# NilsJochem/audio-matcher

Measured on AMD Instinct MI355X. Metric: audio samples/s matched (whole node), 10 s needle vs 1 h haystack, 1/2/4/8 GPU, higher is better.
Workload: dtype f32

## Files before the change

### audio-matcher_amd/csrc/am_context.hip

```cpp
#include "am_internal.h"

namespace am {

thread_local std::string t_err;

int fail(int code, const std::string& msg) {
    t_err = msg;
    return code;
}
int hip_fail(hipError_t e, const char* what) {
    char buf[256];
    snprintf(buf, sizeof(buf), "%s: %s", what, hipGetErrorString(e));
    t_err = buf;
    return e == hipErrorOutOfMemory ? AM_ERR_OOM : AM_ERR_HIP;
}

static std::mutex g_hooks_mu;
static Hooks g_hooks;
Hooks snapshot_hooks() {
    std::lock_guard<std::mutex> lk(g_hooks_mu);
    return g_hooks;
}

using OptRule = const char* (*)(long long& v);
static const char* opt_any(long long&) { return nullptr; }
static const char* opt_bool(long long& v) { v = v ? 1 : 0; return nullptr; }
static const char* opt_log_n(long long& v) { return v != 0 && (v < kLogNMin || v > kLogNMax) ? "log_n out of range" : nullptr; }
static const char* opt_half(long long& v) { v = v <= 0 ? 0 : (v >= 2 ? 2 : 1); return nullptr; }
static const char* opt_every(long long& v) { v = v < 1 ? 1 : v; return nullptr; }
static const char* opt_arm_at(long long& v) { v = v < -1 ? -2 : v; return nullptr; }
static const char* opt_needle_group(long long& v) { return v < 1 || v > kMaxNeedleGroup ? "needle_group out of range" : nullptr; }
static const char* opt_pairs(long long& v) { return v < 1 || v > 64 ? "pairs_per_group out of range" : nullptr; }
static const char* opt_score_norm(long long& v) { return v < 0 || v > 1 ? "score_norm out of range (0 = off, 1 = NCC)" : nullptr; }
static const char* opt_floor_db(long long& v) { return v < 0 || v > 200 ? "score_norm_floor_db out of range (0..200)" : nullptr; }
static const char* opt_distance(long long& v) {
    return v < 0 || v > 3 ? "distance_rule out of range (bit 0: inclusive, bit 1: between plateau starts)" : nullptr;
}
struct Option {
    const char* name;
    std::atomic<long long> value;
    OptRule rule;
    long long Opts::*field;
};
static Option g_options[] = {
    {"log_n", {0}, opt_log_n, &Opts::log_n},
    {"pairs_per_group", {64}, opt_pairs, &Opts::pairs_per_group},
    {"profile_mask", {-1}, opt_any, &Opts::profile_mask},
    {"profile_every", {1}, opt_every, &Opts::profile_every},
    {"half_pipeline", {0}, opt_half, &Opts::half},
    {"batch_overlap", {1}, opt_bool, &Opts::batch_overlap},
    {"needle_group", {8}, opt_needle_group, &Opts::needle_group},
    {"pick_stream_priority", {0}, opt_bool, &Opts::pick_priority},
    {"pick_group", {1}, opt_bool, &Opts::pick_group},
    {"k3_group", {1}, opt_bool, &Opts::k3_group},
    {"host_pick_wait", {1}, opt_bool, &Opts::host_pick_wait},
    {"device_redo", {1}, opt_bool, &Opts::device_redo},
    {"tail_block", {1}, opt_bool, &Opts::tail_block},
    {"dense_scores", {0}, opt_bool, &Opts::dense},
    {"score_norm", {0}, opt_score_norm, &Opts::score_norm},
    {"score_norm_floor_db", {60}, opt_floor_db, &Opts::score_norm_floor_db},
    {"debug_no_realloc", {0}, opt_bool, &Opts::debug_no_realloc},
    {"debug_redo_arm_at", {-2}, opt_arm_at, &Opts::debug_redo_arm_at},
    {"peak_filter_order", {0}, opt_bool, &Opts::peak_filter_order},
    {"distance_rule", {0}, opt_distance, &Opts::distance_rule},
    {"tail_window", {0}, opt_bool, &Opts::tail_window},
    {"surrounding_from", {0}, opt_bool, &Opts::surrounding_from},
};
static Option* find_option(const char* key) {
    for (Option& r : g_options)
        if (!strcmp(key, r.name)) return &r;
    return nullptr;
}

thread_local const Opts* t_opts_pin = nullptr;
Opts snapshot_opts(const am_needle* h) {
    if (t_opts_pin) return *t_opts_pin;
    Opts o;
    for (const Option& r : g_options) o.*r.field = r.value.load(std::memory_order_relaxed);
    if (h && h->opt_log_n >= 0) o.log_n = h->opt_log_n;
    if (h && h->opt_half >= 0) o.half = h->opt_half;
    if (h && h->opt_score_norm >= 0) o.score_norm = h->opt_score_norm;
    return o;
}

thread_local int t_no_realloc = 0;
int realloc_refused(const char* what, size_t bytes, size_t cap) {
    char buf[160];
    snprintf(buf, sizeof(buf), "debug_no_realloc: %s buffer would grow from %zu to %zu bytes while a call is queueing", what, cap, bytes);
    return fail(AM_ERR_HIP, buf);
}

static const char* kKernelNames[] = {"k1_cols_fwd", "k2_rows", "k3_cols_inv", "tile_stats", "peaks", "other"};
static std::mutex g_ctx_mu;
static std::map<int, Ctx*> g_ctx;

int get_ctx(int device, Ctx** out) {
    std::lock_guard<std::mutex> lk(g_ctx_mu);
    int n = 0;
    hipError_t e = hipGetDeviceCount(&n);
    if (e != hipSuccess || n <= 0) return fail(AM_ERR_NO_DEVICE, "no HIP device available");
    if (device < 0 || device >= n) return fail(AM_ERR_NO_DEVICE, "device ordinal out of range");
    auto it = g_ctx.find(device);
    if (it != g_ctx.end()) { *out = it->second; AM_HIP(hipSetDevice(device)); return AM_OK; }
    AM_HIP(hipSetDevice(device));
    (void)hipSetDeviceFlags(hipDeviceScheduleSpin);
    (void)hipGetLastError();
    AM_HIP(fft_kernels_init());
    Ctx* c = new Ctx();
    c->device = device;
    c->hdr.flags = hipHostMallocMapped | hipHostMallocCoherent;
    c->failcnt.flags = hipHostMallocMapped | hipHostMallocCoherent;
    c->spill.flags = hipHostMallocMapped | hipHostMallocCoherent;
    hipError_t se = hipStreamCreateWithFlags(&c->stream, hipStreamNonBlocking);
    if (se != hipSuccess) { delete c; return hip_fail(se, "hipStreamCreate"); }
    {
        int least = 0, greatest = 0;
        if (snapshot_opts(nullptr).pick_priority && hipDeviceGetStreamPriorityRange(&least, &greatest) == hipSuccess && least != greatest)
            (void)hipStreamCreateWithPriority(&c->stream2, hipStreamNonBlocking, least);
        else
            (void)hipStreamCreateWithFlags(&c->stream2, hipStreamNonBlocking);
        (void)hipGetLastError();
    }
    (void)hipStreamCreateWithFlags(&c->stream_tail, hipStreamNonBlocking);
    (void)hipEventCreateWithFlags(&c->ev_fork, kSyncEvent);
    (void)hipEventCreateWithFlags(&c->ev_join, kSyncEvent);
    (void)hipGetLastError();
    for (int i = 0; i < 2; ++i) {
        (void)hipEventCreateWithFlags(&c->ev_k3[i], kSyncEvent);
        (void)hipEventCreateWithFlags(&c->ev_pick[i], kSyncEvent);
    }
    g_ctx[device] = c;
    *out = c;
    return AM_OK;
}

static hipEvent_t prof_event(Ctx* c) {
    if (!c->pool.empty()) { hipEvent_t e = c->pool.back(); c->pool.pop_back(); return e; }
    hipEvent_t e = nullptr;
// ... 445 lines not shown
```

### audio-matcher_amd/csrc/am_correlate.hip

```cpp
#include "am_internal.h"

namespace am {

static int pick_log_n(size_t s, long long out_count, const Opts& o, int* logN_out) {
    int min_log = kLogNMin;
    while (min_log <= kLogNMax && ((size_t)1 << min_log) < s + 1) ++min_log;
    if (min_log > kLogNMax) return fail(AM_ERR_INVALID_ARG, "needle too long for a forced transform size (2^23 at most; leave log_n at 0 for needle partitioning)");
    if (o.log_n > 0) {
        int l = (int)o.log_n;
        if (l < min_log) l = min_log;
        if (l > kLogNMax) l = kLogNMax;
        *logN_out = l;
        return AM_OK;
    }
    const long long span = out_count + (long long)s - 1;
    if (span > (1ll << 19)) {
        if ((long long)s <= kWideFromSamples) { *logN_out = 21; return AM_OK; }
        if ((long long)s <= kWidestFromSamples) {
            long long hop21 = (1ll << 21) - (long long)s + 1;
            if (hop21 >= 8 * kTile) hop21 = (hop21 / kTile) * kTile;
            *logN_out = (hop21 > 0 && out_count <= 2 * hop21) ? 21 : 22;
            return AM_OK;
        }
        if ((long long)s <= kSegmentFrom) {
// ... 154 lines not shown

int run_correlation(am_needle* h, const Opts& o, const void* d_src, long long src_len, long long lead,
                           float* d_dst, long long out_count, float factor,
                           const ScanRequest* scan_req, ScanResult* res, int src_kind, const PassPlan* plan) {
    int rc;
    PassPlan own;
    if (!plan) {
        if ((rc = pass_plan(h, o, out_count, scan_req && !scan_req->no_scan && lead == 0, &own))) return rc;
        plan = &own;
    }
    if (res) { res->fused = false; res->redo_ok = false; res->sparse = plain_scores(); }
    if (plan->kind != PassKind::Partitioned) return run_correlation_one(h, *plan, d_src, src_len, lead, d_dst, out_count, factor, scan_req, res, src_kind, false);
    if (scan_req && scan_req->skip_launch) return fail(AM_ERR_INVALID_ARG, "internal: streaming ingest does not run early pairs for partitioned needles");
    for (size_t i = 0; i < plan->parts.size(); ++i) {
        ScanRequest plain{};
        if (scan_req) {
            plain.margin = -1.0f; plain.range_a = scan_req->range_a; plain.range_b = scan_req->range_b;
            plain.before_k3 = i == 0 ? scan_req->before_k3 : nullptr;
            plain.no_scan = true;
        }
        if ((rc = run_correlation_one(h->segments[i], plan->parts[i], d_src, src_len, lead - h->seg_off[i], d_dst, out_count, factor,
                                      scan_req ? &plain : nullptr, nullptr, src_kind, i > 0)))
            return rc;
    }
    return AM_OK;
}

static int run_correlation_one(am_needle* h, const PassPlan& pp, const void* d_src, long long src_len, long long lead,
                               float* d_dst, long long out_count, float factor,
                               const ScanRequest* scan_req, ScanResult* res, int src_kind, bool accumulate) {
    Ctx* c = h->ctx;
    Job job{};
    job.src = d_src; job.src_len = src_len; job.lead = lead; job.src_kind = src_kind;
    job.dst = d_dst; job.out_count = out_count;
    if (pp.kind == PassKind::Direct) {
        ProfScope ps(c, KN_OTHER);
        AM_HIP(launch_direct(c->stream, job, h->d_needle, (int)h->n, factor));
        return AM_OK;
    }
    int rc;
    const PlanDev& pl = pp.pl->dev;
    const HalfScale& hs = pp.hs;
    const TailPlan& tail = pp.tail;
    const long long N = pp.g.N, hop = pp.g.hop, npairs = pp.npairs, ppg = pp.ppg;
    const ScanBuffers out = (scan_req && scan_req->out.work) ? scan_req->out : scan_buffers(c->side[0]);
    DevBuf& wk = *out.work;
    if ((rc = wk.ensure((size_t)ppg * (size_t)N * sizeof(float2)))) return rc;
    ScanCfg scan{};
    bool fused = false;
    if (scan_req && !scan_req->no_scan) {
        if (res) res->sparse = SparseScores{nullptr, nullptr, nullptr, (int)hop, pl.logN2, pl.logN1, 1.0 / (double)hop};
        if (pp.fused) {
            const long long side_blocks = std::max(pp.g.nblocks, scan_req->side_nblocks);
            if ((rc = out.stats32->ensure((size_t)((out_count + 31) / 32) * sizeof(float2)))) return rc;
            if ((rc = out.wflags->ensure(sparse_bytes(side_blocks, pl)))) return rc;
            fill_scan_cfg(&scan, out.stats32->p, out.wflags->p, side_blocks, pl, scan_req->margin, scan_req->hist_min, scan_req->seg_c, scan_req->seg_d);
            fused = true;
            if (res) { res->fused = true; res->sparse = sparse_view(scan, hop, pl); }
        }
    }
    const float k3scale = hs.k3(factor);
    job.out_count = pp.main_count; job.hop = (int)hop; job.nblocks = (int)pp.nblocks;
    if (scan_req && scan_req->skip_launch) return AM_OK;
    long long pair_lo = 0, pair_hi = npairs;
    bool with_tail = tail.on;
    if (scan_req && scan_req->range_b > scan_req->range_a) {
        pair_lo = (scan_req->range_a / hop) / 2;
        pair_hi = std::min(npairs, ((scan_req->range_b - 1) / hop) / 2 + 1);
        with_tail = tail.on && scan_req->range_b > tail.T;
    }
    if (scan_req && scan_req->tail_by_caller) with_tail = false;
    if (with_tail) {
        AM_HIP(hipEventRecord(c->ev_fork, c->stream));
        AM_HIP(hipStreamWaitEvent(c->stream_tail, c->ev_fork, 0));
        if ((rc = run_tail_block(c, pp, d_src, src_len, d_dst, out_count, factor, scan, src_kind))) return rc;
        AM_HIP(hipEventRecord(c->ev_join, c->stream_tail));
    }
    bool waited = false;
    for (long long first = pair_lo; first < pair_hi; first += ppg) {
        const int np = (int)std::min(ppg, pair_hi - first);
        job.first_pair = (int)first;
        { ProfScope ps(c, KN_K1); AM_HIP(launch_k1(c->stream, job, np, (float2*)wk.p, pl, hs.level)); }
        { ProfScope ps(c, KN_K2); AM_HIP(launch_k2(c->stream, np, (float2*)wk.p, pp.hc, pl, nullptr, hs.level, hs.hscale, hs.pre)); }
        if (!waited && scan_req && scan_req->before_k3) AM_HIP(hipStreamWaitEvent(c->stream, scan_req->before_k3, 0));
        waited = true;
        { ProfScope ps(c, KN_K3); AM_HIP(launch_k3(c->stream, job, np, (const float2*)wk.p, pl, k3scale, scan, hs.level, accumulate)); }
    }
    if (with_tail) AM_HIP(hipStreamWaitEvent(c->stream, c->ev_join, 0));
    if (res && fused && !accumulate && pair_lo == 0 && pair_hi == npairs && npairs <= ppg) {
        res->redo_ok = true;
        job.first_pair = 0;
        res->redo_job = job; res->redo_pl = pl; res->redo_scale = k3scale; res->redo_half = hs.level;
        res->redo_npairs = (int)npairs; res->redo_work = (const float2*)wk.p; res->redo_cfg = scan;
    }
    return AM_OK;
}

float scale_factor(const am_needle* h, int scale, size_t w) {
    if (scale == AM_SCALE_LIB) return h->inv_autocorr;
    if (scale == AM_SCALE_MY) return h->inv_autocorr / (float)w;
    return 1.0f;
}

static uint64_t start_nanos(uint64_t start, uint32_t sr) {
    const double t = (double)start / (double)sr;
    if (!(t > 0.0)) return 0;
    int e = 0;
    const double m = std::frexp(t, &e);
    const unsigned long long mant = (unsigned long long)std::ldexp(m, 53);
    const int sh = e - 53;
    unsigned __int128 v = (unsigned __int128)mant * 1000000000ull;
    if (sh >= 0) return (uint64_t)(v << sh);
    const int r = -sh;
    if (r >= 127) return 0;
    unsigned __int128 q = v >> r;
    const unsigned __int128 rem = v & (((unsigned __int128)1 << r) - 1);
    const unsigned __int128 half = (unsigned __int128)1 << (r - 1);
    if (rem > half || (rem == half && (q & 1))) ++q;
    return (uint64_t)q;
}

static bool is_overshadowed(const am_peak& element, const am_peak* other, uint32_t sr, double max_distance_s) {
    if (!other) return false;
    uint64_t e = start_nanos(element.start, sr), b = start_nanos(other->start, sr);
    if (e < b) std::swap(e, b);
    const uint64_t maxd = (uint64_t)std::llround(max_distance_s * 1e9);
    return (e - b) < maxd && other->prominence > element.prominence;
}

int upload_segments(Ctx* c, const std::vector<Segment>& segs) {
    const size_t bytes = sizeof(Segment) * segs.size();
    if (c->segs.p && segs.size() == c->segs_resident.size() &&
        memcmp(segs.data(), c->segs_resident.data(), bytes) == 0)
        return AM_OK;
    int rc;
    c->segs_resident.clear();
    if ((rc = c->segs.ensure(bytes))) return rc;
    if ((rc = c->pinned.ensure(bytes))) return rc;
    memcpy(c->pinned.p, segs.data(), bytes);
    AM_HIP(hipMemcpyAsync(c->segs.p, c->pinned.p, bytes, hipMemcpyHostToDevice, c->stream));
    AM_HIP(hipStreamSynchronize(c->stream));
    c->segs_resident = segs;
    return AM_OK;
}

int prepare_results(Ctx* c, size_t nhdr, size_t arena_entries, PeakArena* arena) {
    const size_t hdr_bytes = (sizeof(SegHeader) * nhdr + 63) / 64 * 64;
    int rc;
    if ((rc = c->hdr.ensure(hdr_bytes + sizeof(am_peak) * arena_entries))) return rc;
    if ((rc = c->arena_cur.ensure(sizeof(unsigned)))) return rc;
    AM_HIP(hipMemsetAsync(c->arena_cur.p, 0, sizeof(unsigned), c->stream));
    arena->base = reinterpret_cast<am_peak*>(static_cast<char*>(c->hdr.p) + hdr_bytes);
    arena->cursor = static_cast<unsigned*>(c->arena_cur.p);
    arena->cap = (unsigned)arena_entries;
    return AM_OK;
}

int wide_reserve(Ctx* c, size_t n) {
    int rc;
    if ((rc = c->wide_ctl.ensure(n * kWideCtlBytes))) return rc;
    if ((rc = c->wide_list.ensure(n * AM_MAX_PEAKS_PER_CHUNK * sizeof(am_peak)))) return rc;
    return c->wide_tiles.ensure(n * kWideTileList * sizeof(int));
}
WideState wide_carve(Ctx* c, size_t n) {
    WideState wide{};
    wide.best = static_cast<unsigned long long*>(c->wide_ctl.p);
    wide.state = reinterpret_cast<int*>(wide.best + n);
// ... 172 lines not shown
```

### audio-matcher_amd/csrc/am_engine.hip

```cpp
#include "am_internal.h"

namespace am {

static int launch_pick_group(Ctx* c, const K3Group& kg, long long n_scores, int seg_off, int nsegs, float min_prom, long long min_dist,
                             const SparseScores& sp_common, int* bad, const int* hdr_off, const PeakArena& arena, const PeakPolicy& pol,
                             hipStream_t st) {
    if (nsegs == 0 || n_scores <= 0 || kg.n <= 0) return AM_OK;
    int rc;
    const size_t nz = (size_t)kg.n, total = nz * (size_t)nsegs;
    const long long ntiles = (n_scores + kTile - 1) / kTile;
    PickGroup pg{};
    pg.n = kg.n;
    for (int z = 0; z < kg.n; ++z) {
        if ((rc = c->grp_stats[z].ensure((size_t)ntiles * sizeof(float2)))) return rc;
        pg.g[z] = kg.dst[z]; pg.stats[z] = static_cast<float2*>(c->grp_stats[z].p);
        pg.stats32[z] = kg.stats32[z]; pg.wbits[z] = kg.wbits[z]; pg.theta[z] = kg.tile_theta[z];
        pg.hdr_off[z] = hdr_off[z];
    }
    { ProfScope ps(c, KN_STATS, st);
      AM_HIP(launch_stats_reduce(st, pg.stats32[0], n_scores, pg.stats[0], bad, &pg)); }
    if ((rc = wide_reserve(c, total))) return rc;
    if ((rc = c->side[0].peaks.ensure(total * AM_MAX_PEAKS_PER_CHUNK * sizeof(am_peak)))) return rc;
    {
        ProfScope ps(c, KN_PEAKS, st);
        AM_HIP(launch_peaks(st, pg.g[0], n_scores, pg.stats[0], (const Segment*)c->segs.p + seg_off, nsegs, min_prom, min_dist,
                            (am_peak*)c->side[0].peaks.p, (SegHeader*)c->hdr.p, sp_common, arena, wide_carve(c, total), false, pol, &pg));
    }
    return AM_OK;
}


struct ChunkPlan {
    std::vector<Segment> segs, short_segs;
    std::vector<size_t> widths, short_w;
    std::vector<int> seg_off, short_off;
    std::vector<int> n_chunks;
    size_t max_scores = 0, max_segs = 1;
    int ns(size_t k) const { return seg_off[k + 1] - seg_off[k]; }
    bool too_many(size_t nn) const { return max_segs > (size_t)1 << 18 || segs.size() * nn > (size_t)1 << 24; }
};
static void plan_chunks(size_t s, const void* const* d_hays, const size_t* lens, size_t n_hay, const am_match_params* p, const Opts& o,
                        bool split_short, size_t max_windows, ChunkPlan* cp) {
    const size_t window = (size_t)(p->chunk + p->overlap);
    cp->seg_off.assign(n_hay + 1, 0);
    cp->short_off.assign(n_hay + 1, 0);
    cp->n_chunks.assign(n_hay, 0);
    for (size_t k = 0; k < n_hay; ++k) {
        cp->seg_off[k] = (int)cp->segs.size();
        cp->short_off[k] = (int)cp->short_segs.size();
        if (!d_hays[k] || lens[k] < s) continue;
        std::vector<Segment> one;
        std::vector<size_t> w1;
        make_segments(lens[k], s, p, o.tail_window != 0, one, &w1, max_windows);
        cp->n_chunks[k] = (int)one.size();
        for (size_t i = 0; i < one.size(); ++i) {
            const bool shorter = split_short && w1[i] != window;
            (shorter ? cp->short_segs : cp->segs).push_back(one[i]);
            (shorter ? cp->short_w : cp->widths).push_back(w1[i]);
        }
        if (!one.empty()) cp->max_scores = std::max(cp->max_scores, lens[k] - s + 1);
        cp->max_segs = std::max(cp->max_segs, cp->segs.size() - (size_t)cp->seg_off[k]);
    }
    cp->seg_off[n_hay] = (int)cp->segs.size();
    cp->short_off[n_hay] = (int)cp->short_segs.size();
}

struct ScoreSets {
    Ctx* c;
    bool overlap;
    size_t seq = 0;
    ScoreSets(Ctx* c_, const Opts& o, size_t n_items)
        : c(c_), overlap(o.batch_overlap && n_items > 1 && c_->stream2 && c_->ev_k3[0] && c_->ev_k3[1] && c_->ev_pick[0] && c_->ev_pick[1]) {}
    int count() const { return overlap ? 2 : 1; }
    int set() const { return overlap ? (int)(seq & 1) : 0; }
    ScoreSide& side() const { return c->side[set()]; }
    float* scores() const { return (float*)side().scores.p; }
    hipStream_t pick_stream() const { return overlap ? c->stream2 : c->stream; }
    int size(size_t max_scores, size_t max_segs) {
        int rc;
        for (int set = 0; set < count(); ++set) {
            ScoreSide& sd = c->side[set];
            if ((rc = sd.scores.ensure(max_scores * sizeof(float)))) return rc;
            if ((rc = sd.peaks.ensure(sizeof(am_peak) * max_segs * AM_MAX_PEAKS_PER_CHUNK))) return rc;
            if ((rc = sd.stats.ensure((max_scores + kTile - 1) / kTile * sizeof(float2)))) return rc;
        }
        return wide_reserve(c, max_segs);
    }
    int wait_pick(bool on_host) {
        if (!overlap || seq < 2) return AM_OK;
        if (on_host) AM_HIP(hipEventSynchronize(c->ev_pick[set()]));
        else AM_HIP(hipStreamWaitEvent(c->stream, c->ev_pick[set()], 0));
        return AM_OK;
    }
    int k3_done() {
        if (!overlap) return AM_OK;
        AM_HIP(hipEventRecord(c->ev_k3[set()], c->stream));
        AM_HIP(hipStreamWaitEvent(c->stream2, c->ev_k3[set()], 0));
        return AM_OK;
    }
    int pick_done() {
        if (overlap) AM_HIP(hipEventRecord(c->ev_pick[set()], c->stream2));
        ++seq;
        return AM_OK;
    }
    int drain() {
        AM_HIP(hipStreamSynchronize(c->stream));
        if (overlap) AM_HIP(hipStreamSynchronize(c->stream2));
        return AM_OK;
    }
};

static int match_alone(am_needle* h, const void* d_hay, size_t len, const am_match_params* p, am_peak* out, size_t cap, size_t slot,
                       size_t* n_out, int src_kind, const PartSpec* part, int* worst) {
    const int rc = match_many(h, &d_hay, &len, 1, p, out ? out + slot * cap : nullptr, cap, &n_out[slot], src_kind, 0, 1, false, nullptr, part);
    if (rc == AM_ERR_CAPACITY) *worst = rc;
    return rc == AM_ERR_CAPACITY ? AM_OK : rc;
}

static int pick_alone(am_needle* h, const Opts& o, const am_match_params* p, const void* src, long long src_len, float factor,
                      const ScanRequest& req, long long n_scores, int seg_idx, const Segment& sg, int spare_hdr, uint64_t shift, int src_kind,
                      const NormSpec& nrm, std::vector<am_peak>& all) {
    Ctx* c = h->ctx;
    const PeakPolicy pol = o.peak_policy();
    int rc;
    PeakArena own{};
    if ((rc = c->spill.ensure(sizeof(am_peak) * AM_MAX_PEAKS_PER_CHUNK))) return rc;
    AM_HIP(hipMemsetAsync(c->arena_cur.p, 0, sizeof(unsigned), c->stream));
    own.base = static_cast<am_peak*>(c->spill.p); own.cursor = static_cast<unsigned*>(c->arena_cur.p);
    own.cap = AM_MAX_PEAKS_PER_CHUNK;
    ScoreSide& side = c->side[0];
    if ((rc = side.scores.ensure((size_t)n_scores * sizeof(float)))) return rc;
    float* d_scores = (float*)side.scores.p;
    ScanResult res{};
    if ((rc = run_correlation(h, o, src, src_len, 0, d_scores, n_scores, factor, &req, &res, src_kind))) return rc;
    if (nrm.on) {
        if ((rc = normalise_scores(c, c->stream, nrm, src, src_len, src_kind, 0, (long long)h->n, d_scores, sg.a, std::min(sg.b, n_scores))))
            return rc;
        res.fused = false;
    }
    if ((rc = launch_pick(c, side, d_scores, n_scores, seg_idx, 1, p->min_prominence, (long long)p->min_distance, nullptr, &res, spare_hdr, own, pol))) return rc;
    AM_HIP(hipStreamSynchronize(c->stream));
    const SegHeader& hd = static_cast<const SegHeader*>(c->hdr.p)[spare_hdr];
    const size_t old = all.size();
    if (hd.overflow & 1) {
        if ((rc = pick_chunk_big(c, d_scores, n_scores, seg_idx, sg, p->min_prominence, (long long)p->min_distance, &res, hd.seg_min, all, pol)))
            return rc;
    } else append_header_peaks(hd, own, all);
    for (size_t j = old; j < all.size(); ++j) { all[j].start += shift; all[j].end += shift; }
    return AM_OK;
}

struct TailSlots { size_t scores, stats; };
static bool tail_batchable(const TailPlan& t) { return t.on && t.g.logN == 21; }
static int launch_tail_batch(am_needle* h, const std::vector<PassPlan>& plans, const std::vector<size_t>& members, int half_idx,
                             const TailSlots& sl, const void* const* d_hays, const size_t* lens, float factor, int src_kind) {
    Ctx* c = h->ctx;
    const PassPlan& lead = plans[members[0]];
    const TailPlan& first = lead.tail;
    const Plan* pl = lead.tail_pl;
    const float2* hc = lead.tail_hc;
    const HalfScale& hs = lead.tail_hs;
    TailBatch tb{};
    tb.n = (int)members.size();
    for (int j = 0; j < tb.n; ++j) {
        const size_t k = members[j];
        const size_t slot = (size_t)half_idx * kMaxTailBatch + (size_t)j;
        const Job job = tail_job(plans[k].tail, d_hays[k], (long long)lens[k], (long long)(lens[k] - h->n + 1), src_kind);
        tb.src[j] = job.src;
        tb.src_len[j] = job.src_len;
        tb.out_count[j] = job.out_count;
        tb.dst[j] = static_cast<float*>(c->tail_scores.p) + slot * sl.scores;
        tb.stats32[j] = static_cast<float2*>(c->tail_stats.p) + slot * sl.stats;
    }
    float2* work = static_cast<float2*>(c->work_tail.p);
    { ProfScope ps(c, KN_OTHER); AM_HIP(launch_tail_batch_k1(c->stream, tb, (int)first.g.hop, src_kind, work, pl->dev, hs.level)); }
    { ProfScope ps(c, KN_OTHER); AM_HIP(launch_k2(c->stream, tb.n, work, hc, pl->dev, nullptr, hs.level, hs.hscale, hs.pre, true)); }
    { ProfScope ps(c, KN_OTHER); AM_HIP(launch_tail_batch_k3(c->stream, tb, (int)first.g.hop, work, pl->dev, hs.k3(factor), hs.level)); }
    return AM_OK;
}

static int classify_nonfinite(am_needle* h, const PassPlan& pp, const float* d_hay, size_t len,
                              const std::vector<Segment>& segs, int s0, int s1,
                              std::vector<char>* drop, std::vector<char>* again) {
    Ctx* c = h->ctx;
    const long long s = (long long)h->n;
    const int nch = s1 - s0;
    drop->assign(nch, 0); again->assign(nch, 0);
    std::vector<Segment> ranges;
    for (int i = s0; i < s1; ++i)
        ranges.push_back(Segment{segs[i].a, std::min<long long>((long long)len, segs[i].b + s - 1)});
    const long long npairs = pp.kind == PassKind::Transform ? pp.npairs : 0;
    for (long long q = 0; q < npairs; ++q) ranges.push_back(pp.pair_reads(q, (long long)len));
    if (pp.tail.on) ranges.push_back(pp.tail_reads((long long)len));
    std::vector<int> flags(ranges.size(), 0);
    int rc = nonfinite_flags(c, d_hay, ranges.data(), (int)ranges.size(), flags.data());
    if (rc) return rc;
    for (int i = 0; i < nch; ++i) {
        if (flags[i]) { (*drop)[i] = 1; continue; }
        if (pp.kind == PassKind::Partitioned) { (*again)[i] = 1; continue; }
        const Segment sg = segs[s0 + i];
        for (long long q = 0; q < npairs && !(*again)[i]; ++q)
            if (flags[nch + q] && 2 * q * pp.g.hop < sg.b && (2 * q + 2) * pp.g.hop > sg.a) (*again)[i] = 1;
        if (pp.tail.on && flags[nch + npairs] && pp.tail.T < sg.b) (*again)[i] = 1;
    }
    return AM_OK;
}

int match_many(am_needle* h, const void* const* d_hays, const size_t* lens, size_t n_hay,
               const am_match_params* p, am_peak* out, size_t cap_per_hay, size_t* n_out, int src_kind,
               size_t index_base, size_t index_stride, bool fire_hooks, const StreamPre* pre, const PartSpec* part) {
    Ctx* c = h->ctx;
    const Opts o = snapshot_opts(h);
    const PeakPolicy pol = o.peak_policy();
    Hooks hooks = fire_hooks ? snapshot_hooks() : Hooks{};
    if (part) hooks.fn = nullptr;
    if (part && n_hay != 1) return fail(AM_ERR_INVALID_ARG, "internal: a part is one haystack");
    auto G = [&](size_t k) { return index_base + k * index_stride; };
    const size_t s = h->n;
    if (p->chunk == 0) return fail(AM_ERR_INVALID_ARG, "chunk must be > 0");
    if (p->scale < AM_SCALE_NONE || p->scale > AM_SCALE_MY) return fail(AM_ERR_INVALID_ARG, "bad scale");
    const NormSpec nrm = norm_spec(h, o);
    if (nrm.on && (pre || part)) return fail(AM_ERR_INVALID_ARG, AM_NORM_UNSUPPORTED);
    int rc = norm_check(nrm, p->scale);
    if (rc) return rc;
    const bool my = p->scale == AM_SCALE_MY;
    const float factor = nrm.on ? norm_factor(nrm) : scale_factor(h, p->scale, (size_t)(p->chunk + p->overlap));
    const int sm = p->scale == AM_SCALE_LIB ? 1 : 0;
    ScanRequest base{};
    base.margin = nrm.on ? -1.0f : write_margin(o, p);
    const bool sparse_ok = base.margin >= 0.0f;
    base.hist_min = nrm.on ? FLT_MAX : h->hist_min(sm);
    base.seg_c = (long long)p->chunk;
    base.seg_d = (long long)(p->chunk + p->overlap) - (long long)s;
    for (size_t k = 0; k < n_hay; ++k) n_out[G(k)] = 0;
    ChunkPlan cp;
    plan_chunks(s, d_hays, lens, n_hay, p, o, my, part ? part->max_windows : (size_t)-1, &cp);
    const std::vector<Segment>& segs = cp.segs;
    const std::vector<int>& seg_off = cp.seg_off;
    const size_t nsegs = segs.size();
    if (nsegs == 0 && cp.short_segs.empty()) return AM_OK;
    if (cp.too_many(1)) return fail(AM_ERR_INVALID_ARG, "chunk size too small for this haystack (more than 2^18 chunks)");
    size_t n_active = 0;
    for (size_t k = 0; k < n_hay; ++k) n_active += cp.ns(k) > 0;
    ScoreSets sets(c, o, n_active);
    if ((rc = sets.size(cp.max_scores, cp.max_segs))) return rc;
    std::vector<PassPlan> plans(n_hay);
    Footprint need;
    for (size_t k = 0; k < n_hay; ++k) {
        if (cp.n_chunks[k] == 0 || cp.ns(k) == 0) continue;
        if ((rc = pass_plan(h, o, (long long)(lens[k] - s + 1), pre == nullptr, &plans[k]))) return rc;
        need.take(plans[k].need);
    }
    std::vector<int> tail_slot(n_hay, -1);
    TailSlots tslots{0, 0};
    bool batch_tails = false;
    if (need.work_tail) {
        size_t n_tails = 0;
        for (size_t k = 0; k < n_hay; ++k)
            if (tail_batchable(plans[k].tail)) {
                ++n_tails;
                tslots.scores = std::max(tslots.scores, (size_t)(2 * plans[k].tail.g.hop));
            }
        tslots.stats = tslots.scores / 32;
        batch_tails = sets.overlap && n_tails > 1;
        const size_t nslot = batch_tails ? kMaxTailBatch : 1;
        if ((rc = c->work_tail.ensure(need.work_tail * nslot))) return rc;
        if (batch_tails) {
            if ((rc = c->tail_scores.ensure(2 * kMaxTailBatch * tslots.scores * sizeof(float)))) return rc;
            if ((rc = c->tail_stats.ensure(2 * kMaxTailBatch * tslots.stats * sizeof(float2)))) return rc;
        }
    }
    int tail_batches = 0;
    for (int set = 0; set < sets.count(); ++set) {
        if (need.work && (rc = c->side[set].work.ensure(need.work))) return rc;
        if (pre) continue;
        if (need.stats32 && (rc = c->side[set].stats32.ensure(need.stats32))) return rc;
        if (need.side && (rc = c->side[set].wflags.ensure(need.side))) return rc;
    }
    PeakArena arena{};
    if ((rc = prepare_results(c, nsegs + 1, std::min<size_t>(cp.max_segs * AM_MAX_PEAKS_PER_CHUNK, (size_t)1 << 20) + nsegs * 8, &arena))) return rc;
    std::vector<Segment> resident = segs;
    for (const Segment& sg : cp.short_segs) resident.push_back(Segment{0, sg.b - sg.a});
    const int local_seg = (int)resident.size();
    resident.push_back(Segment{0, std::max<long long>(base.seg_d + 1, 1)});
    if ((rc = upload_segments(c, resident))) return rc;
    if ((rc = c->badflag.ensure(sizeof(int) * n_hay))) return rc;
    int* h_bad = static_cast<int*>(c->badflag.p);
    memset(h_bad, 0, sizeof(int) * n_hay);
    if ((rc = c->failcnt.ensure(nsegs + 1))) return rc;
    if (nrm.on) {
        size_t max_len = 0;
        for (size_t k = 0; k < n_hay; ++k) if (cp.ns(k) > 0) max_len = std::max(max_len, lens[k]);
        if ((rc = norm_reserve(c, (long long)max_len))) return rc;
    }
    unsigned char* h_fail = static_cast<unsigned char*>(c->failcnt.p);
    memset(h_fail, 0, nsegs + 1);
    const bool device_redo = sets.overlap && sparse_ok && !needle_is_segmented(h, o) && o.device_redo != 0;
    if (device_redo) {
        for (int set = 0; set < 2; ++set)
            if ((rc = c->redo_pairs[set].ensure(sizeof(int) * (size_t)std::max<long long>(need.npairs, 1)))) return rc;
    }
    SegHeader* h_hdr = static_cast<SegHeader*>(c->hdr.p);
    auto chunk_events = [&](size_t k, int stage) {
        if (hooks.chunk_fn)
            for (int i = 0; i < cp.n_chunks[k]; ++i)
                hooks.chunk_fn(hooks.chunk_user, G(k), (part ? part->chunk_base : 0) + (size_t)i,
                               part ? part->chunk_total : (size_t)cp.n_chunks[k], stage);
    };
    const bool arm_forced = o.debug_redo_arm_at >= -1;
    bool redo_armed = device_redo && (arm_forced ? o.debug_redo_arm_at == 0 : h->redo_armed_left[sm] > 0);
    QueueingScope queueing(o.debug_no_realloc != 0);
    for (size_t k = 0; k < n_hay; ++k) {
        const int ns = cp.ns(k);
        if (cp.n_chunks[k] == 0) continue;
        if (device_redo && arm_forced) redo_armed = o.debug_redo_arm_at >= 0 && (long long)k >= o.debug_redo_arm_at;
        else if (device_redo && !redo_armed && (k & 3) == 0) {
            const volatile unsigned char* f = h_fail;
            for (int i = 0; i < seg_off[k] && !redo_armed; ++i) redo_armed = f[i] != 0;
        }
        if (hooks.fn) hooks.fn(hooks.user, G(k), 0, (size_t)cp.n_chunks[k]);
        chunk_events(k, 0);
        if (ns == 0) continue;
        const long long out_count = (long long)(lens[k] - s + 1);
        const int set = sets.set();
        const PassPlan& pp = plans[k];
        ScoreSide& side = sets.side();
        float* d_scores = sets.scores();
        ScanRequest req = base;
        req.out = scan_buffers(side);
        if ((rc = sets.wait_pick(o.host_pick_wait != 0))) return rc;
        int* d_redo = nullptr;
        if (redo_armed) {
            AM_HIP(hipMemsetAsync(c->redo_pairs[set].p, 0, sizeof(int) * (size_t)std::max<long long>(pp.g.npairs, 1), c->stream));
            d_redo = static_cast<int*>(c->redo_pairs[set].p);
        }
        int* bad = ((src_kind == 0 || o.half) && std::isfinite(factor)) ? &h_bad[k] : nullptr;
        if (pre) {
            d_scores = pre->scores;
            req.out.stats32 = pre->stats32; req.out.wflags = pre->side;
            req.side_nblocks = pre->layout_nblocks;
            req.range_a = std::min(pre->pairs_done, pp.g.npairs) * 2 * pp.g.hop;
            req.range_b = out_count;
            req.skip_launch = req.range_a >= out_count;
        }
        if (batch_tails && tail_batchable(pp.tail)) {
            if (tail_slot[k] < 0) {
                std::vector<size_t> members;
                for (size_t k2 = k; k2 < n_hay && members.size() < (size_t)kMaxTailBatch; ++k2)
                    if (tail_batchable(plans[k2].tail) && tail_slot[k2] < 0) {
                        tail_slot[k2] = (tail_batches & 1) * kMaxTailBatch + (int)members.size();
                        members.push_back(k2);
                    }
                if ((rc = launch_tail_batch(h, plans, members, tail_batches & 1, tslots, d_hays, lens, factor, src_kind))) return rc;
                ++tail_batches;
            }
            req.tail_by_caller = true;
        }
        ScanResult res{};
        if ((rc = run_correlation(h, o, d_hays[k], (long long)lens[k], 0, d_scores, out_count, factor, &req, &res, src_kind, &pp))) return rc;
        if ((rc = sets.k3_done())) return rc;
        if (req.tail_by_caller && res.fused) {
            const TailPlan& t = pp.tail;
            const BallotLayout bl = ballot_layout(res.sparse.log_n1, res.sparse.log_n2);
            const size_t blk = (size_t)(t.T / res.sparse.hop);
            ProfScope ps(c, KN_OTHER, c->stream2);
            AM_HIP(launch_tail_commit(c->stream2, static_cast<const float*>(c->tail_scores.p) + (size_t)tail_slot[k] * tslots.scores, d_scores + t.T,
                                      out_count - t.T, static_cast<const float2*>(c->tail_stats.p) + (size_t)tail_slot[k] * tslots.stats,
                                      const_cast<float2*>(res.sparse.stats32) + t.T / 32,
                                      res.sparse.wbits ? const_cast<unsigned long long*>(res.sparse.wbits) + blk * bl.words : nullptr, (long long)bl.words,
                                      res.sparse.tile_theta ? const_cast<float*>(res.sparse.tile_theta) + blk * bl.tiles : nullptr, (int)bl.tiles));
        }
        if (res.fused && res.sparse.wbits) {
            res.sparse.fail_flags = h_fail + seg_off[k];
            res.sparse.redo_pairs = (redo_armed && res.redo_ok) ? d_redo : nullptr;
        }
        if (nrm.on) {
            if ((rc = normalise_scores(c, sets.pick_stream(), nrm, d_hays[k], (long long)lens[k], src_kind, 0, (long long)s, d_scores, 0, out_count)))
                return rc;
        }
        if ((rc = launch_pick(c, side, d_scores, out_count, seg_off[k], ns, p->min_prominence,
                              (long long)p->min_distance, bad, nrm.on ? nullptr : &res, seg_off[k], arena, pol, sets.pick_stream()))) return rc;
        if (res.fused && res.sparse.redo_pairs) {
            ScanCfg cfg = res.redo_cfg;
            cfg.margin = -1.0f;
            cfg.only_pairs = d_redo;
            { ProfScope ps(c, KN_OTHER, c->stream2);
              AM_HIP(launch_k3(c->stream2, res.redo_job, res.redo_npairs, res.redo_work, res.redo_pl, res.redo_scale, cfg, res.redo_half)); }
            res.sparse.redo_pairs = nullptr; res.sparse.fail_flags = nullptr;
            if ((rc = launch_pick(c, side, d_scores, out_count, seg_off[k], ns, p->min_prominence, (long long)p->min_distance,
                                  nullptr, &res, seg_off[k], arena, pol, c->stream2, true))) return rc;
        }
        if ((rc = sets.pick_done())) return rc;
    }
    queueing.end();
    if ((rc = sets.drain())) return rc;
    int worst = AM_OK;
    std::vector<am_peak> all;
    std::vector<size_t> retry_f32;
    const int spare_hdr = (int)nsegs;
    for (size_t k = 0; k < n_hay; ++k) {
        const int s0 = seg_off[k], s1 = seg_off[k + 1];
        if (cp.n_chunks[k] == 0) continue;
        const long long out_count = (long long)(lens[k] - s + 1);
        if (h_bad[k] && o.half) { retry_f32.push_back(k); continue; }
        if (!my && !nrm.on && !h_bad[k] && s1 > s0) {
            std::vector<float> mins;
            int failed = 0;
            for (int i = s0; i < s1; ++i) { mins.push_back(h_hdr[i].seg_min); failed += h_fail[i] != 0; }
            std::sort(mins.begin(), mins.end());
            if (failed * 8 > s1 - s0) h->conservative_left[sm] = 64;
            const bool robust = device_redo && h->conservative_left[sm] == 0;
            h->remember_min(sm, robust ? mins[mins.size() / 2] : mins.front());
            if (h->conservative_left[sm] > 0) --h->conservative_left[sm];
            if (failed) h->redo_armed_left[sm] = 64;
            else if (h->redo_armed_left[sm] > 0) --h->redo_armed_left[sm];
        }
        all.clear();
        std::vector<char> drop, again;
        if (h_bad[k]) {
            if ((rc = classify_nonfinite(h, plans[k], (const float*)d_hays[k], lens[k], segs, s0, s1, &drop, &again))) return rc;
        }
        for (int i = s0; i < s1; ++i) {
            if (!drop.empty() && drop[i - s0]) continue;
            const Segment sg = segs[i];
            if (!again.empty() && again[i - s0]) {
                ScanRequest one{};
                one.margin = -1.0f;
                if ((rc = pick_alone(h, o, p, advance_src(d_hays[k], (size_t)sg.a), (long long)cp.widths[i], factor, one, sg.b - sg.a,
                                     local_seg, Segment{0, sg.b - sg.a}, spare_hdr, (uint64_t)sg.a, src_kind, nrm, all))) return rc;
                continue;
            }
            if (!(h_hdr[i].overflow & 7)) { append_header_peaks(h_hdr[i], arena, all); continue; }
            ScanRequest full = base;
            full.margin = -1.0f;
            full.range_a = sg.a; full.range_b = sg.b;
            if ((rc = pick_alone(h, o, p, d_hays[k], (long long)lens[k], factor, full, out_count, i, sg, spare_hdr, 0, src_kind, nrm, all))) return rc;
        }
        for (int i = cp.short_off[k]; i < cp.short_off[k + 1]; ++i) {
            const Segment sg = cp.short_segs[i];
            ScanRequest one{};
            one.margin = -1.0f;
            if ((rc = pick_alone(h, o, p, advance_src(d_hays[k], (size_t)sg.a), (long long)cp.short_w[i], scale_factor(h, p->scale, cp.short_w[i]),
                                 one, sg.b - sg.a, (int)nsegs + i, Segment{0, sg.b - sg.a}, spare_hdr, (uint64_t)sg.a, src_kind, nrm, all))) return rc;
        }
        if (part) {
            for (am_peak& q : all) { q.start += part->first_sample; q.end += part->first_sample; }
            part->raw->insert(part->raw->end(), all.begin(), all.end());
            n_out[G(k)] = all.size();
            rc = AM_OK;
        } else rc = merge_peaks(all, p, o.surrounding_from != 0, out ? out + G(k) * cap_per_hay : nullptr, cap_per_hay, &n_out[G(k)]);
        chunk_events(k, 1);
        if (hooks.fn) hooks.fn(hooks.user, G(k), 1, (size_t)cp.n_chunks[k]);
        if (rc == AM_ERR_CAPACITY) worst = rc;
        else if (rc) return rc;
    }
    for (size_t k : retry_f32) {
        const long long keep = h->opt_half;
        h->opt_half = 0;
        rc = match_alone(h, d_hays[k], lens[k], p, out, cap_per_hay, G(k), n_out, src_kind, part, &worst);
        h->opt_half = keep;
        chunk_events(k, 1);
        if (hooks.fn) hooks.fn(hooks.user, G(k), 1, (size_t)cp.n_chunks[k]);
        if (rc) return rc;
    }
    return worst;
}

int match_multi_many(am_needle* const* needles, size_t nn, const void* const* d_hays, const size_t* lens, size_t n_hay,
                     int src_kind, const am_match_params* p, am_peak* out, size_t cap_per_pair, size_t* n_out,
                     size_t index_base, size_t index_stride, const uint64_t* overlaps, bool varlen) {
    am_needle* h0 = needles[0];
    Ctx* c = h0->ctx;
    const Opts o = snapshot_opts(h0);
    const PeakPolicy pol = o.peak_policy();
    const Hooks hooks = snapshot_hooks();
    auto G = [&](size_t k) { return index_base + k * index_stride; };
    for (size_t j = 0; j < nn; ++j) {
        if (!needles[j] || needles[j]->ctx != c) return fail(AM_ERR_INVALID_ARG, "needles must live on one device");
        if (!varlen && needles[j]->n != h0->n) return fail(AM_ERR_INVALID_ARG, "am_match_multi: needles must have equal length");
    }
    if (o.score_norm) return fail(AM_ERR_INVALID_ARG, AM_NORM_UNSUPPORTED);
    if (p->chunk == 0) return fail(AM_ERR_INVALID_ARG, "chunk must be > 0");
    if (p->scale != AM_SCALE_NONE && p->scale != AM_SCALE_LIB)
        return fail(AM_ERR_INVALID_ARG, "am_match_multi supports AM_SCALE_NONE and AM_SCALE_LIB");
    for (size_t k = 0; k < n_hay; ++k)
        for (size_t j = 0; j < nn; ++j) n_out[G(k) * nn + j] = 0;
    std::vector<am_match_params> pj(nn, *p);
    if (overlaps)
        for (size_t j = 0; j < nn; ++j) pj[j].overlap = overlaps[j];
    int rc, worst = AM_OK;
    std::vector<size_t> ord;
    bool any_segmented = false;
    for (size_t j = 0; j < nn; ++j) {
        if (needle_is_segmented(needles[j], o)) any_segmented = true;
        else ord.push_back(j);
    }
    if (any_segmented)
        for (size_t k = 0; k < n_hay; ++k)
            for (size_t j = 0; j < nn; ++j)
                if (needle_is_segmented(needles[j], o) &&
                    (rc = match_alone(needles[j], d_hays[k], lens[k], &pj[j], out, cap_per_pair, G(k) * nn + j, n_out, src_kind, nullptr, &worst)))
                    return rc;
    if (ord.empty()) return worst;
    std::stable_sort(ord.begin(), ord.end(), [&](size_t a, size_t b) { return needles[a]->n > needles[b]->n; });
    const size_t m = ord.size();
    const size_t s = needles[ord[0]]->n;
    const size_t s_min = needles[ord[m - 1]]->n;
    const int sm = p->scale == AM_SCALE_LIB ? 1 : 0;
    std::vector<ChunkPlan> cps;
    std::vector<std::pair<size_t, uint64_t>> keys;
    std::vector<int> plan_of(m), seg_base, hdr_base(m);
    for (size_t i = 0; i < m; ++i) {
        const size_t j = ord[i];
        const std::pair<size_t, uint64_t> key(needles[j]->n, pj[j].overlap);
        const size_t u = (size_t)(std::find(keys.begin(), keys.end(), key) - keys.begin());
        if (u == keys.size()) {
            keys.push_back(key);
            cps.emplace_back();
            plan_chunks(key.first, d_hays, lens, n_hay, &pj[j], o, false, (size_t)-1, &cps.back());
        }
        plan_of[i] = (int)u;
    }
    std::vector<Segment> all_segs;
    size_t max_scores = 0, max_segs = 1, nhdr = 0;
    bool too_many = false;
    for (const ChunkPlan& cpu : cps) {
        seg_base.push_back((int)all_segs.size());
        all_segs.insert(all_segs.end(), cpu.segs.begin(), cpu.segs.end());
        max_scores = std::max(max_scores, cpu.max_scores);
        max_segs = std::max(max_segs, cpu.max_segs);
        too_many = too_many || cpu.too_many(1);
    }
    for (size_t i = 0; i < m; ++i) { hdr_base[i] = (int)nhdr; nhdr += cps[plan_of[i]].segs.size(); }
    if (nhdr == 0) return worst;
    if (too_many || nhdr > (size_t)1 << 24) return fail(AM_ERR_INVALID_ARG, "chunk size too small for this batch (too many chunks)");
    auto plan_i = [&](size_t i) -> const ChunkPlan& { return cps[plan_of[i]]; };
    auto seg_of = [&](size_t k, size_t i) { return seg_base[plan_of[i]] + plan_i(i).seg_off[k]; };
    auto hdr_of = [&](size_t k, size_t i) { return hdr_base[i] + plan_i(i).seg_off[k]; };
// ... 254 lines not shown
```

### audio-matcher_amd/csrc/am_internal.h

```cpp
#pragma once
#include <algorithm>
#include <atomic>
#include <cfloat>
#include <cmath>
#include <cstdio>
#include <cstring>
#include <map>
#include <mutex>
#include <string>
#include <vector>

#include "am_kernels.h"
#include "am_spans.h"

namespace am {

extern thread_local std::string t_err;
int fail(int code, const std::string& msg);
int hip_fail(hipError_t e, const char* what);
#define AM_HIP(call)                                         \
    do {                                                     \
        hipError_t e_ = (call);                              \
        if (e_ != hipSuccess) return hip_fail(e_, #call);    \
    } while (0)

struct Hooks {
    am_progress_fn fn = nullptr;
    void* user = nullptr;
    am_chunk_progress_fn chunk_fn = nullptr;
    void* chunk_user = nullptr;
};
Hooks snapshot_hooks();

struct Opts {
    long long log_n, pairs_per_group, half, batch_overlap, needle_group, dense, device_redo, debug_no_realloc, debug_redo_arm_at;
    long long peak_filter_order, distance_rule, tail_window, surrounding_from, k3_group, pick_group, tail_block, host_pick_wait;
    long long profile_mask, profile_every, pick_priority;
    long long score_norm, score_norm_floor_db;
    PeakPolicy peak_policy() const { return PeakPolicy{(int)peak_filter_order, (int)(distance_rule & 1), (int)((distance_rule >> 1) & 1)}; }
};
static const float kHalfGain = 1024.0f;
static const double kMinEfficiency = 0.75;
static const int kLogNMin = 10, kLogNMax = 23;
static const long long kWideFromSamples = 140000;
static const long long kWidestFromSamples = 1500000;
static const long long kSegmentFrom = 1ll << 22;
static const long long kSegmentLen = 1ll << 22;

extern thread_local int t_no_realloc;
struct QueueingScope {
    bool on;
    explicit QueueingScope(bool enable) : on(enable) { if (on) ++t_no_realloc; }
    ~QueueingScope() { end(); }
    void end() { if (on) { --t_no_realloc; on = false; } }
    QueueingScope(const QueueingScope&) = delete;
    QueueingScope& operator=(const QueueingScope&) = delete;
};
int realloc_refused(const char* what, size_t bytes, size_t cap);

struct DevBuf {
    void* p = nullptr;
    size_t cap = 0;
    int ensure(size_t bytes) {
        if (bytes <= cap) return AM_OK;
        if (t_no_realloc > 0) return realloc_refused("a device", bytes, cap);
        release();
        size_t want = bytes + bytes / 8;
        hipError_t e = hipMalloc(&p, want);
        if (e != hipSuccess) {
            e = hipMalloc(&p, bytes);
            want = bytes;
            if (e != hipSuccess) { p = nullptr; return hip_fail(e, "hipMalloc(scratch)"); }
        }
        cap = want;
        return AM_OK;
    }
    void release() {
        if (p) (void)hipFree(p);
        p = nullptr; cap = 0;
    }
};
struct HostBuf {
    void* p = nullptr;
    size_t cap = 0;
    unsigned flags = hipHostMallocDefault;
    int ensure(size_t bytes) {
        if (bytes <= cap) return AM_OK;
        if (t_no_realloc > 0) return realloc_refused("a pinned host", bytes, cap);
        release();
        hipError_t e = hipHostMalloc(&p, bytes, flags);
        if (e != hipSuccess) { p = nullptr; return hip_fail(e, "hipHostMalloc"); }
        cap = bytes;
        return AM_OK;
    }
    void release() {
        if (p) (void)hipHostFree(p);
        p = nullptr; cap = 0;
    }
};

struct Plan {
    PlanDev dev{};
    float2* tables = nullptr;
    unsigned* mf = nullptr;
};

struct ScoreSide { DevBuf scores, stats, stats32, wflags, peaks, work; };

struct ProfRec { int name; hipEvent_t e0, e1; };
enum { KN_K1 = 0, KN_K2, KN_K3, KN_STATS, KN_PEAKS, KN_OTHER, KN_COUNT };

struct Ctx {
    int device = -1;
    hipStream_t stream = nullptr;
    hipStream_t stream2 = nullptr;
    hipStream_t stream_tail = nullptr;
    hipEvent_t ev_fork = nullptr, ev_join = nullptr;
    DevBuf work_tail, tail_scores, tail_stats;
    DevBuf work_tail2;
    std::recursive_mutex mu;
    std::map<int, Plan> plans;
    ScoreSide side[2];
    DevBuf work2, segs, io_in, io_out, sum, arena_cur, wide_ctl, wide_list, wide_tiles;
    DevBuf norm_blk;
    DevBuf hit_tab, hit_parts, hit_flags, hit_out, hit_stage;
    HostBuf hit_io;
    std::map<int, DevBuf> band_tabs;
    DevBuf warp_tab, warp_needles;
    DevBuf sig_span, sig_scores, sig_psum, sig_pmax, sig_mean, sig_hmax;
    std::map<std::pair<int, int>, DevBuf> rs_taps;
    DevBuf lag_parts, lag_r;
    DevBuf redo_pairs[2];
    DevBuf grp_scores[2][kMaxNeedleGroup], grp_stats32[2][kMaxNeedleGroup], grp_wflags[2][kMaxNeedleGroup];
    DevBuf grp_stats[kMaxNeedleGroup];
    HostBuf failcnt;
    hipEvent_t ev_k3[2] = {nullptr, nullptr}, ev_pick[2] = {nullptr, nullptr};
    HostBuf pinned;
    HostBuf hdr;
    HostBuf spill;
    HostBuf badflag;
    DevBuf ranges, range_flags;
    DevBuf big;
    DevBuf best_stats, best_lmax, best_ctl, best_trans, best_list, best_scores, best_mono;
    std::vector<Segment> segs_resident;
    bool prof = false;
    std::vector<ProfRec> pending;
    std::vector<hipEvent_t> pool;
    double prof_ms[KN_COUNT] = {0};
    uint64_t prof_n[KN_COUNT] = {0};
    uint64_t prof_seq[KN_COUNT] = {0};
};

#ifndef AM_EVENT_NO_SYSTEM_FENCE
#define AM_EVENT_NO_SYSTEM_FENCE 1
#endif
constexpr unsigned kSyncEvent = hipEventDisableTiming | (AM_EVENT_NO_SYSTEM_FENCE ? hipEventDisableSystemFence : 0u);

int get_ctx(int device, Ctx** out);
struct ProfScope {
    Ctx* c; int name; hipStream_t st; hipEvent_t e0 = nullptr, e1 = nullptr;
    bool on;
    ProfScope(Ctx* c_, int name_, hipStream_t st_ = nullptr);
    ~ProfScope() {
        if (on) { (void)hipEventRecord(e1, st); c->pending.push_back({name, e0, e1}); }
    }
};
hipError_t copy_on_stream(Ctx* c, void* dst, const void* src, size_t bytes, hipMemcpyKind kind);
int get_plan(Ctx* c, int logN, const Plan** out, int force_logN1 = 0);

}

struct am_needle {
    am::Ctx* ctx = nullptr;
    float* d_needle = nullptr;
    size_t n = 0;
    float inv_autocorr = 0.f;
    double energy = 0.0;
    std::map<int, float2*> spectra;
    std::map<int, unsigned*> spectra16;
    std::map<int, unsigned*> spectra16m;
    static constexpr int kRecent = 8;
    float recent_min[2][kRecent];
    int recent_n[2] = {0, 0}, recent_pos[2] = {0, 0};
    void remember_min(int sm, float v) {
        recent_min[sm][recent_pos[sm]] = v;
        recent_pos[sm] = (recent_pos[sm] + 1) % kRecent;
        if (recent_n[sm] < kRecent) ++recent_n[sm];
    }
    int conservative_left[2] = {0, 0};
    int redo_armed_left[2] = {0, 0};
    float hist_min(int sm) const {
        float m = FLT_MAX;
        for (int i = 0; i < recent_n[sm]; ++i) m = std::min(m, recent_min[sm][i]);
        return m;
    }
    long long opt_log_n = -1, opt_half = -1, opt_score_norm = -1;
    std::vector<am_needle*> segments;
    std::vector<long long> seg_off;
    bool owns_data = true;
};

namespace am {

struct ScanBuffers { DevBuf* work; DevBuf* stats32; DevBuf* wflags; };
inline ScanBuffers scan_buffers(ScoreSide& sd) { return ScanBuffers{&sd.work, &sd.stats32, &sd.wflags}; }
struct ScanRequest {
    float margin;
    float hist_min;
    long long seg_c, seg_d;
    ScanBuffers out;
    hipEvent_t before_k3;
    long long range_a, range_b;
    long long side_nblocks;
    bool skip_launch;
    bool tail_by_caller;
    bool no_scan;
};
struct ScanResult {
    bool fused;
    SparseScores sparse;
    bool redo_ok;
    Job redo_job; PlanDev redo_pl; float redo_scale; int redo_half; int redo_npairs; const float2* redo_work; ScanCfg redo_cfg;
};
inline SparseScores plain_scores() { return SparseScores{nullptr, nullptr, nullptr, 1, 5, 5, 1.0}; }
struct Geometry {
    int logN;
    long long N, hop, nblocks, npairs;
};
struct TailPlan {
    bool on;
    long long T;
    Geometry g;
};
struct HalfScale {
    int level;
    float pre, hscale;
    float k3(float factor) const { return level ? factor / (hscale * pre) : factor; }
};
struct Footprint {
    size_t work = 0, stats32 = 0, side = 0, work_tail = 0;
    long long npairs = 0;
    void take(const Footprint& f) {
        work = std::max(work, f.work); stats32 = std::max(stats32, f.stats32); side = std::max(side, f.side);
        work_tail = std::max(work_tail, f.work_tail);
        npairs = std::max(npairs, f.npairs);
    }
};
enum class PassKind { Direct, Partitioned, Transform };
struct PassPlan {
    PassKind kind = PassKind::Direct;
    Geometry g{};
    const Plan* pl = nullptr;
    const float2* hc = nullptr;
    HalfScale hs{};
    bool fused = false;
    TailPlan tail{};
    const Plan* tail_pl = nullptr;
    const float2* tail_hc = nullptr;
    HalfScale tail_hs{};
    long long nblocks = 0, npairs = 0;
    long long ppg = 0;
    long long main_count = 0;
    std::vector<PassPlan> parts;
    Footprint need;
    Segment pair_reads(long long q, long long len) const {
        const long long last_block = (2 * q + 1 < nblocks) ? 2 * q + 1 : 2 * q;
        return Segment{2 * q * g.hop, std::min(len, last_block * g.hop + g.N)};
    }
    Segment tail_reads(long long len) const { return Segment{tail.T, std::min(len, tail.T + (tail.g.nblocks - 1) * tail.g.hop + tail.g.N)}; }
};
struct PartSpec {
    size_t max_windows;
    uint64_t first_sample;
    size_t chunk_base, chunk_total;
    std::vector<am_peak>* raw;
};
struct StreamPre {
    float* scores;
    DevBuf* stats32; DevBuf* side;
    long long pairs_done;
    long long layout_nblocks;
};

inline const void* advance_src(const void* src, size_t elements) {
    return static_cast<const char*>(src) + 4 * elements;
}

Opts snapshot_opts(const am_needle* h);
extern thread_local const Opts* t_opts_pin;
struct OptsPin {
    const Opts* prev;
    explicit OptsPin(const Opts* o) : prev(t_opts_pin) { t_opts_pin = o; }
    ~OptsPin() { t_opts_pin = prev; }
    OptsPin(const OptsPin&) = delete;
// ... 193 lines not shown
```

Before: 229.0 billion.

## Run last batch item's pick on main stream and drain results per item

Adds per-item pick events so the host can consume each haystack's peaks as soon as that item's pick finishes, instead of draining all streams before post-processing. The last active item runs its tail commit, redo and pick on the main stream, skipping the cross-stream handoff, and waits for the previous pick either on the host or via a stream wait. The aim is to overlap host-side peak assembly with remaining device work and cut the tail latency of the batch. The cost is more event bookkeeping, and a fallback drain path is needed for rare overflow and bad-flag cases.

```diff
diff --git a/audio-matcher_amd/csrc/am_context.hip b/audio-matcher_amd/csrc/am_context.hip
--- a/audio-matcher_amd/csrc/am_context.hip
+++ b/audio-matcher_amd/csrc/am_context.hip
@@ -54,6 +54,7 @@
     {"pick_group", {1}, opt_bool, &Opts::pick_group},
     {"k3_group", {1}, opt_bool, &Opts::k3_group},
     {"host_pick_wait", {1}, opt_bool, &Opts::host_pick_wait},
+    {"last_on_main", {1}, opt_bool, &Opts::last_on_main},
     {"device_redo", {1}, opt_bool, &Opts::device_redo},
     {"tail_block", {1}, opt_bool, &Opts::tail_block},
     {"dense_scores", {0}, opt_bool, &Opts::dense},
diff --git a/audio-matcher_amd/csrc/am_correlate.hip b/audio-matcher_amd/csrc/am_correlate.hip
--- a/audio-matcher_amd/csrc/am_correlate.hip
+++ b/audio-matcher_amd/csrc/am_correlate.hip
@@ -260,7 +260,10 @@
         job.first_pair = (int)first;
         { ProfScope ps(c, KN_K1); AM_HIP(launch_k1(c->stream, job, np, (float2*)wk.p, pl, hs.level)); }
         { ProfScope ps(c, KN_K2); AM_HIP(launch_k2(c->stream, np, (float2*)wk.p, pp.hc, pl, nullptr, hs.level, hs.hscale, hs.pre)); }
-        if (!waited && scan_req && scan_req->before_k3) AM_HIP(hipStreamWaitEvent(c->stream, scan_req->before_k3, 0));
+        if (!waited && scan_req && scan_req->before_k3) {
+            if (scan_req->before_k3_host) AM_HIP(hipEventSynchronize(scan_req->before_k3));
+            else AM_HIP(hipStreamWaitEvent(c->stream, scan_req->before_k3, 0));
+        }
         waited = true;
         { ProfScope ps(c, KN_K3); AM_HIP(launch_k3(c->stream, job, np, (const float2*)wk.p, pl, k3scale, scan, hs.level, accumulate)); }
     }
diff --git a/audio-matcher_amd/csrc/am_engine.hip b/audio-matcher_amd/csrc/am_engine.hip
--- a/audio-matcher_amd/csrc/am_engine.hip
+++ b/audio-matcher_amd/csrc/am_engine.hip
@@ -75,7 +75,6 @@
     int set() const { return overlap ? (int)(seq & 1) : 0; }
     ScoreSide& side() const { return c->side[set()]; }
     float* scores() const { return (float*)side().scores.p; }
-    hipStream_t pick_stream() const { return overlap ? c->stream2 : c->stream; }
     int size(size_t max_scores, size_t max_segs) {
         int rc;
         for (int set = 0; set < count(); ++set) {
@@ -86,21 +85,46 @@
         }
         return wide_reserve(c, max_segs);
     }
+    bool per_item = false;
+    int item_events(size_t n_items) {
+        if (!overlap) return AM_OK;
+        while (c->ev_item.size() < n_items) {
+            hipEvent_t e = nullptr;
+            AM_HIP(hipEventCreateWithFlags(&e, hipEventDisableTiming));
+            c->ev_item.push_back(e);
+        }
+        per_item = true;
+        return AM_OK;
+    }
+    hipEvent_t pick_event(size_t i) const { return per_item ? c->ev_item[i] : c->ev_pick[i & 1]; }
+    bool last = false;
+    hipStream_t pick_stream() const { return overlap && !last ? c->stream2 : c->stream; }
+    hipEvent_t begin_last() {
+        if (!overlap || !per_item || seq == 0) return nullptr;
+        last = true;
+        return pick_event(seq - 1);
+    }
     int wait_pick(bool on_host) {
         if (!overlap || seq < 2) return AM_OK;
-        if (on_host) AM_HIP(hipEventSynchronize(c->ev_pick[set()]));
-        else AM_HIP(hipStreamWaitEvent(c->stream, c->ev_pick[set()], 0));
+        if (on_host) AM_HIP(hipEventSynchronize(pick_event(seq - 2)));
+        else AM_HIP(hipStreamWaitEvent(c->stream, pick_event(seq - 2), 0));
         return AM_OK;
     }
     int k3_done() {
-        if (!overlap) return AM_OK;
+        if (!overlap || last) return AM_OK;
         AM_HIP(hipEventRecord(c->ev_k3[set()], c->stream));
         AM_HIP(hipStreamWaitEvent(c->stream2, c->ev_k3[set()], 0));
         return AM_OK;
     }
     int pick_done() {
-        if (overlap) AM_HIP(hipEventRecord(c->ev_pick[set()], c->stream2));
+        if (overlap && !last) AM_HIP(hipEventRecord(pick_event(seq), c->stream2));
         ++seq;
+        return AM_OK;
+    }
+    int wait_item(size_t i) {
+        if (!overlap || !per_item) return drain();
+        if (last && i + 1 == seq) AM_HIP(hipStreamSynchronize(c->stream));
+        else AM_HIP(hipEventSynchronize(c->ev_item[i]));
         return AM_OK;
     }
     int drain() {
@@ -244,6 +268,11 @@
     for (size_t k = 0; k < n_hay; ++k) n_active += cp.ns(k) > 0;
     ScoreSets sets(c, o, n_active);
     if ((rc = sets.size(cp.max_scores, cp.max_segs))) return rc;
+    if ((rc = sets.item_events(n_active))) return rc;
+    std::vector<long long> item_of(n_hay, -1);
+    size_t last_active = n_hay;
+    for (size_t k = 0, i = 0; k < n_hay; ++k)
+        if (cp.ns(k) > 0) { item_of[k] = (long long)i++; last_active = k; }
     std::vector<PassPlan> plans(n_hay);
     Footprint need;
     for (size_t k = 0; k < n_hay; ++k) {
@@ -329,6 +358,10 @@
         ScanRequest req = base;
         req.out = scan_buffers(side);
         if ((rc = sets.wait_pick(o.host_pick_wait != 0))) return rc;
+        if (k == last_active && o.last_on_main && !pre && pp.kind != PassKind::Direct) {
+            req.before_k3 = sets.begin_last();
+            req.before_k3_host = o.host_pick_wait != 0;
+        }
         int* d_redo = nullptr;
         if (redo_armed) {
             AM_HIP(hipMemsetAsync(c->redo_pairs[set].p, 0, sizeof(int) * (size_t)std::max<long long>(pp.g.npairs, 1), c->stream));
@@ -359,12 +392,13 @@
         ScanResult res{};
         if ((rc = run_correlation(h, o, d_hays[k], (long long)lens[k], 0, d_scores, out_count, factor, &req, &res, src_kind, &pp))) return rc;
         if ((rc = sets.k3_done())) return rc;
+        const hipStream_t pst = sets.pick_stream();
         if (req.tail_by_caller && res.fused) {
             const TailPlan& t = pp.tail;
             const BallotLayout bl = ballot_layout(res.sparse.log_n1, res.sparse.log_n2);
             const size_t blk = (size_t)(t.T / res.sparse.hop);
-            ProfScope ps(c, KN_OTHER, c->stream2);
-            AM_HIP(launch_tail_commit(c->stream2, static_cast<const float*>(c->tail_scores.p) + (size_t)tail_slot[k] * tslots.scores, d_scores + t.T,
+            ProfScope ps(c, KN_OTHER, pst);
+            AM_HIP(launch_tail_commit(pst, static_cast<const float*>(c->tail_scores.p) + (size_t)tail_slot[k] * tslots.scores, d_scores + t.T,
                                       out_count - t.T, static_cast<const float2*>(c->tail_stats.p) + (size_t)tail_slot[k] * tslots.stats,
                                       const_cast<float2*>(res.sparse.stats32) + t.T / 32,
                                       res.sparse.wbits ? const_cast<unsigned long long*>(res.sparse.wbits) + blk * bl.words : nullptr, (long long)bl.words,
@@ -384,16 +418,21 @@
             ScanCfg cfg = res.redo_cfg;
             cfg.margin = -1.0f;
             cfg.only_pairs = d_redo;
-            { ProfScope ps(c, KN_OTHER, c->stream2);
-              AM_HIP(launch_k3(c->stream2, res.redo_job, res.redo_npairs, res.redo_work, res.redo_pl, res.redo_scale, cfg, res.redo_half)); }
+            { ProfScope ps(c, KN_OTHER, pst);
+              AM_HIP(launch_k3(pst, res.redo_job, res.redo_npairs, res.redo_work, res.redo_pl, res.redo_scale, cfg, res.redo_half)); }
             res.sparse.redo_pairs = nullptr; res.sparse.fail_flags = nullptr;
             if ((rc = launch_pick(c, side, d_scores, out_count, seg_off[k], ns, p->min_prominence, (long long)p->min_distance,
-                                  nullptr, &res, seg_off[k], arena, pol, c->stream2, true))) return rc;
+                                  nullptr, &res, seg_off[k], arena, pol, pst, true))) return rc;
         }
         if ((rc = sets.pick_done())) return rc;
     }
     queueing.end();
-    if ((rc = sets.drain())) return rc;
+    struct AtRest {
+        ScoreSets& sets; bool done = false;
+        int operator()() { if (done) return AM_OK; done = true; return sets.drain(); }
+        ~AtRest() { if (!done) (void)sets.drain(); }
+    } rest{sets};
+    if (!sets.overlap && (rc = rest())) return rc;
     int worst = AM_OK;
     std::vector<am_peak> all;
     std::vector<size_t> retry_f32;
@@ -401,6 +440,13 @@
     for (size_t k = 0; k < n_hay; ++k) {
         const int s0 = seg_off[k], s1 = seg_off[k + 1];
         if (cp.n_chunks[k] == 0) continue;
+        if (!rest.done && item_of[k] >= 0 && (rc = sets.wait_item((size_t)item_of[k]))) return rc;
+        if (k == last_active) rest.done = true;
+        {
+            bool rare = h_bad[k] != 0 || cp.short_off[k + 1] > cp.short_off[k];
+            for (int i = s0; i < s1 && !rare; ++i) rare = (h_hdr[i].overflow & 7) != 0;
+            if (rare && (rc = rest())) return rc;
+        }
         const long long out_count = (long long)(lens[k] - s + 1);
         if (h_bad[k] && o.half) { retry_f32.push_back(k); continue; }
         if (!my && !nrm.on && !h_bad[k] && s1 > s0) {
@@ -454,6 +500,7 @@
         if (rc == AM_ERR_CAPACITY) worst = rc;
         else if (rc) return rc;
     }
+    if ((rc = rest())) return rc;
     for (size_t k : retry_f32) {
         const long long keep = h->opt_half;
         h->opt_half = 0;
diff --git a/audio-matcher_amd/csrc/am_internal.h b/audio-matcher_amd/csrc/am_internal.h
--- a/audio-matcher_amd/csrc/am_internal.h
+++ b/audio-matcher_amd/csrc/am_internal.h
@@ -35,7 +35,7 @@
 struct Opts {
     long long log_n, pairs_per_group, half, batch_overlap, needle_group, dense, device_redo, debug_no_realloc, debug_redo_arm_at;
     long long peak_filter_order, distance_rule, tail_window, surrounding_from, k3_group, pick_group, tail_block, host_pick_wait;
-    long long profile_mask, profile_every, pick_priority;
+    long long profile_mask, profile_every, pick_priority, last_on_main;
     long long score_norm, score_norm_floor_db;
     PeakPolicy peak_policy() const { return PeakPolicy{(int)peak_filter_order, (int)(distance_rule & 1), (int)((distance_rule >> 1) & 1)}; }
 };
@@ -135,6 +135,7 @@
     DevBuf grp_stats[kMaxNeedleGroup];
     HostBuf failcnt;
     hipEvent_t ev_k3[2] = {nullptr, nullptr}, ev_pick[2] = {nullptr, nullptr};
+    std::vector<hipEvent_t> ev_item;
     HostBuf pinned;
     HostBuf hdr;
     HostBuf spill;
@@ -210,6 +211,7 @@
     long long seg_c, seg_d;
     ScanBuffers out;
     hipEvent_t before_k3;
+    bool before_k3_host;
     long long range_a, range_b;
     long long side_nblocks;
     bool skip_launch;
```

New measurement: 226.0 billion. 0.987x the previous value.
